# pqh22/ProxyTransformation

Hardware: AMD Instinct MI355X
Metric: scenes/sec (100k pts, 256 clusters, 64 proxies) (higher is better)
Workload: dtype f32; 1 GPU; cfg2: N=100000 pts, gs=8->M'=256 kept clusters, L=64 text + V=196 image proxies, d=256, eval forward; scenes_per_gpu=4, img_feat_dtype=bf16, input_sets_rotated=3, streams=1, lanes=1 (one forward at a time), setup_forwards=32

## Files before the change

### proxytransformation_amd/csrc/api.hip

```cpp
#include <atomic>
#include <chrono>
#include <cmath>
#include <cstdlib>
#include <cstring>
#include <mutex>
#include <utility>
#include <vector>

#include "common.h"

namespace ptx {

static thread_local char g_err[512] = "";

void set_error(const char *fmt, ...)
{
    va_list ap;
    va_start(ap, fmt);
    vsnprintf(g_err, sizeof(g_err), fmt, ap);
    va_end(ap);
}

static const char *const kKernelNames[] = {
    "k_minmax", "k_cluster", "k_select", "k_tags",
// ... 377 lines not shown
                         float *img_proxy, void *ws, hipStream_t st, int phase = 0, bool need_ln = true,
                         int i0 = 0, int ni = -1, uint32_t *gate = nullptr, uint32_t gate_seq = 0)
{
    const PrepLayout P = prep_layout(s);
    const WsLayout L = ws_layout(s);
    const int C = s.C, hd = P.hd, nall = s.B * s.V, nimg = ni < 0 ? nall : ni;
    float *fm = at<float>(ws, L.fm) + (size_t)i0 * s.in_dim, *qkv0 = at<float>(ws, L.qkv0) + (size_t)i0 * 3 * C;
    float *we = at<float>(ws, L.we) + (size_t)i0 * s.heads * P.KT1, *gbuf = at<float>(ws, L.gbuf) + (size_t)i0 * s.heads * P.KT2p;
    float *obuf = at<float>(ws, L.obuf) + (size_t)i0 * C, *cbuf = at<float>(ws, L.cbuf) + (size_t)i0 * C;
    if (img_proxy) img_proxy += (size_t)i0 * C;
    const int dt = s.img_dtype;
    img = static_cast<const char *>(img) + (size_t)i0 * s.in_dim * s.hw * (dt == 0 ? 4 : 2);
    float *Gs = nullptr, *E = nullptr, *ML = nullptr;
    const int EW = P.KT2p - s.in_dim;
    const bool pooled32 = img_pool32_supported(dt, s.in_dim, s.hw, s.heads);
    const bool pooled = pooled32 || img_pool_supported(dt, s.in_dim, s.hw, s.heads);
    if (pooled) {
        img_pool_layout(at<float>(ws, L.pool), nall, s.in_dim, EW, &Gs, &E, &ML);
        Gs += (size_t)i0 * 2 * s.heads * s.in_dim; E += (size_t)i0 * s.heads * EW; ML += (size_t)i0 * s.heads * 5;
    }
    if (phase != 2) PTX_TIMED(KID_IMG_MEAN, st, launch_img_mean(img, dt, nimg, s.in_dim, s.hw, fm, st, gate, gate_seq));
    if (phase == 1) return PTX_OK;
    const bool chained = hd == 32 && nimg < 4096;
    {
        GemmBatch g{}; g.n = 1;
        g.p[0] = GemmProb{fm, prep + P.w3, qkv0, prep + P.b3, nullptr, nullptr, nullptr,
                          nimg, 3 * C, s.in_dim, s.in_dim, s.in_dim, 3 * C, 0, 0, 0, EPI_NONE};
        if (chained) {
            g.p[0].w2 = prep + P.t1; g.p[0].c2 = we; g.p[0].n2 = P.KT1; g.p[0].ldc2 = s.heads * P.KT1;
            g.p[0].chain_tiles = s.heads; g.p[0].w2_stride = (long)P.KT1 * hd; g.p[0].c2_stride = P.KT1;
        }
        PTX_TIMED(KID_IMG_QKV0, st, launch_gemm(g, st));
    }
    if (!chained) {
        for (int h0 = 0; h0 < s.heads; h0 += kMaxGroups) {
            GemmBatch g{}; g.n = std::min(kMaxGroups, s.heads - h0);
            for (int h = h0; h < h0 + g.n; ++h)
                g.p[h - h0] = GemmProb{qkv0 + h * hd, prep + P.t1 + (size_t)h * P.KT1 * hd, we + (size_t)h * P.KT1,
                                       nullptr, nullptr, nullptr, nullptr, nimg, P.KT1, hd, 3 * C, hd,
                                       s.heads * P.KT1, 0, 0, 0, EPI_NONE};
            PTX_TIMED(KID_IMG_WE, st, launch_gemm(g, st));
        }
    }
    if (pooled32) {
        PTX_TIMED_EXT(KID_IMG_SCORES, st, launch_img_pool32(static_cast<const float *>(img), we, qkv0, nimg, s.in_dim, s.hw, C, P.KT1, EW,
                                                        attn_scale(hd), Gs, E, ML, st));
    } else if (pooled) {
        PTX_TIMED_EXT(KID_IMG_SCORES, st, launch_img_pool(img, dt, we, qkv0, nimg, s.in_dim, s.hw, C, P.KT1,
                                                      EW, attn_scale(hd), Gs, E, ML, st));
    } else {
        PTX_TIMED(KID_IMG_SCORES, st, launch_img_scores(img, dt, we, qkv0, nimg, s.in_dim, s.hw, s.heads, C, P.KT1,
                                                        P.KT2p, attn_scale(hd), gbuf, st));
        PTX_TIMED(KID_IMG_GATHER, st, launch_img_gather(img, dt, nimg, s.in_dim, s.hw, s.heads, P.KT2p, gbuf, st));
    }
    for (int h0 = 0; h0 < s.heads; h0 += kMaxGroups) {
        GemmBatch g{}; g.n = std::min(kMaxGroups, s.heads - h0);
        for (int h = h0; h < h0 + g.n; ++h) {
            GemmProb &gp = g.p[h - h0];
            gp = GemmProb{gbuf + (size_t)h * P.KT2p, prep + P.t2 + (size_t)h * hd * P.KT2p, obuf + h * hd,
                          w.v_b + h * hd, nullptr, gbuf + (size_t)h * P.KT2p + s.in_dim,
                          qkv0 + 2 * C + h * hd, nimg, hd, P.KT2p, s.heads * P.KT2p, P.KT2p, C,
                          0, s.heads * P.KT2p, 3 * C, EPI_NONE};
            if (pooled) {
                gp.A = nullptr; gp.rs = nullptr;
                gp.pg = Gs + (size_t)h * s.in_dim; gp.ldg = 2 * s.heads * s.in_dim; gp.gslab = s.heads * s.in_dim;
                gp.pe = E + (size_t)h * EW; gp.lde = s.heads * EW;
                gp.pml = ML + (size_t)h * 5; gp.ldml = s.heads * 5;
                gp.kg = s.in_dim;
            }
        }
        PTX_TIMED(KID_IMG_O, st, launch_gemm(g, st));
    }
    {
        GemmBatch g{}; g.n = 1;
        g.p[0] = GemmProb{obuf, w.c_w, cbuf, w.c_b, nullptr, nullptr, nullptr,
                          nimg, C, C, C, C, C, 0, 0, 0, EPI_NONE};
        g.p[0].lnp_out = at<float>(ws, L.lnp_img) + (size_t)i0 * (C / 32) * 2;
        PTX_TIMED(KID_IMG_C, st, launch_gemm(g, st));
    }
    if (need_ln) {
        LnBatch lb{}; lb.n = 1; lb.C = C; lb.eps = s.ln_eps;
        lb.p[0] = LnProb{cbuf, img_proxy, w.norm_img_w, w.norm_img_b, nullptr, nimg, 1};
        PTX_TIMED(KID_IMG_LN, st, launch_ln_rows(lb, st));
    }
    return PTX_OK;
}

struct Branch {
    const PtxBlock *blk; const float *x_in; const float *proxy; int Lp; const uint8_t *mask;
    const float *head_w, *head_b, *head_ab; int nout; float *head_out; float *guide; int slot;
    bool late_proxy;
// ... 797 lines not shown
```

### proxytransformation_amd/csrc/common.h

```cpp
#pragma once
#include <hip/hip_runtime.h>
#include <cstdarg>
#include <cstdint>
#include <cstdio>

#include "../../include/proxyt.h"

namespace ptx {

void set_error(const char *fmt, ...);
bool timing_ext_take(hipEvent_t *start, hipEvent_t *stop);

#define PTX_REQUIRE(cond, ...)                                   \
    do {                                                         \
        if (!(cond)) {                                           \
            ::ptx::set_error(__VA_ARGS__);                       \
            return PTX_EINVAL;                                   \
        }                                                        \
    } while (0)

#define PTX_HIP(expr)                                                              \
    do {                                                                           \
        hipError_t e_ = (expr);                                                    \
        if (e_ != hipSuccess) {                                                    \
// ... 188 lines not shown
    size_t order, picks, keep, ksrc, kcenter, kcluster, kidx, drop_idx, tile_counts;
    size_t point_proxy, x_in[2];
    size_t pp_all, xln_all[2], g_all[2];
    size_t order_e;
    size_t fm, qkv0, we, pool, gbuf, obuf, cbuf, img_proxy;
    size_t qkv[2], pt[2], pv[2], ao[2], x1[2], xn2[2], hbuf[2], x2[2], guide[2], head[2];
    size_t lnp_img, lnp_x1[2];
    size_t fa_part;
    size_t mlp_part;
    size_t total;
};
WsLayout ws_layout(const PtxShape &s);

int validate_shape(const PtxShape &s);

enum : int { EPI_NONE = 0, EPI_GELU = 1 };
struct GemmProb {
    const float *A; const float *W; float *C;
    const float *bias;
    const float *res;
    const float *rs;
    const float *ad;
    int R, N, K, lda, ldw, ldc, ldres, rs_stride, ldad, epi;
    const float *pg, *pe, *pml; int ldg, gslab, lde, ldml, kg;
    float *lnp_out;
    const float *lnp_in, *ln_c; int ln_parts, ln_C; float ln_eps;
    const float *w2; float *c2; int n2, ldc2, chain_tiles; long w2_stride, c2_stride;
};
constexpr int kMaxGroups = 8;
struct GemmBatch {
    GemmProb p[kMaxGroups]; int n; int rotate;
    GateRef tail_gate;
};
int launch_gemm(const GemmBatch &gb, hipStream_t st, int compute_dtype = 0);
int gemm_policy(int min_tiles_128);

struct LnProb { const float *x; float *y; const float *w; const float *b; const float *add; int R, add_rows; };
struct LnBatch { LnProb p[2]; int n; int C; float eps; };
int launch_ln_rows(const LnBatch &lb, hipStream_t st);

struct HeadProb {
    const float *x; const float *nw; const float *nb;
    const float *hw; const float *hb;
    const float *ab;
    float *out; float *guide; int R, nout;
};
struct HeadBatch { HeadProb p[2]; int n; int C; float eps; };
// ... 70 lines not shown
                const int32_t *keep = nullptr);
int launch_select_slots(const PtxShape &s, const int32_t *idx, const float *cluster, const int32_t *order,
                        const int32_t *picks, const int32_t *keep, float *kcluster, int32_t *kidx,
                        int32_t *drop_idx, uint32_t *tag, hipStream_t st);
int launch_t_ln_fwd(const float *x, const float *w, const float *b, int R, int C, float eps, float *y, float *stats, hipStream_t st);
int t_ln_chunks(int R);
int launch_t_ln_bwd(const float *x, const float *stats, const float *w, const float *dy, int R, int C, float *dx, float *part, hipStream_t st);
int launch_tile_count(const uint32_t *tag, int B, int N, int32_t *tile_counts, int32_t *counts, int32_t *scene_acc,
                      hipStream_t st);
int launch_affine(const PtxShape &s, const ScenePts &points, uint32_t *tag, const float *kcenter,
                  const float *translate, const float *transform, float *out, int32_t *counts,
                  const int32_t *tile_counts, bool compact, bool clear_tag, hipStream_t st,
                  const uint32_t *poison = nullptr);

int launch_img_mean(const void *img, int dt, int nimg, int in_dim, int hw, float *fm, hipStream_t st,
                    uint32_t *gate = nullptr, uint32_t gate_seq = 0);
int launch_img_scores(const void *img, int dt, const float *we, const float *qkv0, int nimg, int in_dim,
                      int hw, int heads, int C, int KT1, int KT2p, float scale, float *gbuf, hipStream_t st);
int launch_img_gather(const void *img, int dt, int nimg, int in_dim, int hw, int heads, int KT2p, float *gbuf,
                      hipStream_t st);
bool img_pool_supported(int dt, int in_dim, int hw, int heads);
size_t img_pool_bytes(int nimg, int in_dim, int EW);
void img_pool_layout(float *scratch, int nimg, int in_dim, int EW, float **Gs, float **E, float **ML);
int launch_img_pool(const void *img, int dt, const float *we, const float *qkv0, int nimg, int in_dim, int hw, int C,
                    int KT1, int EW, float scale, float *Gs, float *E, float *ML, hipStream_t st);

bool img_pool32_supported(int dt, int in_dim, int hw, int heads);
int launch_img_pool32(const float *img, const float *we, const float *qkv0, int nimg, int in_dim, int hw, int C, int KT1, int EW,
                      float scale, float *Gs, float *E, float *ML, hipStream_t st);

int run_prepare(const PtxShape &s, const PtxWeights &w, float *prep, hipStream_t st);

}
```

### proxytransformation_amd/csrc/gemm.hip

```cpp
#include <atomic>
#include <cstdlib>

#include "common.h"
#include "split3.h"
#include "mfma64.h"

namespace ptx {


__device__ __forceinline__ void pin4(float4 &v) { asm volatile("" : "+v"(v.x), "+v"(v.y), "+v"(v.z), "+v"(v.w)); }
__device__ __forceinline__ void ln_row_stats(const GemmProb &pr, int row, float &mu, float &rstd)
{
    const float2 *pp = reinterpret_cast<const float2 *>(pr.lnp_in) + (size_t)row * pr.ln_parts;
    constexpr int kMaxParts = 16;
    float2 v[kMaxParts];
#pragma unroll
    for (int t = 0; t < kMaxParts; ++t) v[t] = pp[min(t, pr.ln_parts - 1)];
    float s1 = 0.0f, s2 = 0.0f;
#pragma unroll
    for (int t = 0; t < kMaxParts; ++t) { s1 += t < pr.ln_parts ? v[t].x : 0.0f; s2 += t < pr.ln_parts ? v[t].y : 0.0f; }
    const float inv = 1.0f / (float)pr.ln_C;
    mu = s1 * inv;
    float between = 0.0f;
#pragma unroll
// ... 449 lines not shown
#undef PTX_Y_COMPUTE

template <int SK, int AMODE, bool CHAIN = false, bool LN = false>
__global__ __launch_bounds__(SK * 64) void k_gemm32(GemmBatch gb)
{
    const GemmProb pr = gb.p[blockIdx.z];
    const int row0 = blockIdx.x * 32, col0 = blockIdx.y * 32;
    if (row0 >= pr.R || col0 >= pr.N) return;
    extern __shared__ __attribute__((aligned(16))) float lds[];
    const int lane = threadIdx.x & 63;
    const int wv = __builtin_amdgcn_readfirstlane(threadIdx.x >> 6);
    float *base = lds + (size_t)wv * (4 * 32 * LDT);
    const int li = lane & 31, hh = lane >> 5;
    const int nk = (pr.K + BK - 1) / BK, per = (nk + SK - 1) / SK;
    const int it0 = wv * per, it1 = min(nk, it0 + per);
    const int r0 = lane >> 3, kq = (lane & 7) * 4;
    const size_t a0 = (size_t)min(row0 + r0, pr.R - 1) * pr.lda, a1 = (size_t)min(row0 + r0 + 8, pr.R - 1) * pr.lda;
    const size_t a2 = (size_t)min(row0 + r0 + 16, pr.R - 1) * pr.lda, a3 = (size_t)min(row0 + r0 + 24, pr.R - 1) * pr.lda;
    const size_t w0 = (size_t)min(col0 + r0, pr.N - 1) * pr.ldw, w1 = (size_t)min(col0 + r0 + 8, pr.N - 1) * pr.ldw;
    const size_t w2 = (size_t)min(col0 + r0 + 16, pr.N - 1) * pr.ldw, w3 = (size_t)min(col0 + r0 + 24, pr.N - 1) * pr.ldw;
    const float4 z4 = make_float4(0.f, 0.f, 0.f, 0.f);
    float4 aA0, aA1, aA2, aA3, wA0, wA1, wA2, wA3, aB0, aB1, aB2, aB3, wB0, wB1, wB2, wB3;
    float4 gA0 = z4, gA1 = z4, gA2 = z4, gA3 = z4, gB0 = z4, gB1 = z4, gB2 = z4, gB3 = z4;
    int kA = 0, kB = 0;
    (void)kA; (void)kB;
    size_t g0 = 0, g1 = 0, g2 = 0, g3 = 0, e0 = 0, e1 = 0, e2 = 0, e3 = 0;
    float fc0[4] = {0.f, 0.f, 0.f, 0.f}, fc1[4] = {0.f, 0.f, 0.f, 0.f}, fct[4] = {0.f, 0.f, 0.f, 0.f};
    float *cts = lds + (size_t)SK * (4 * 32 * LDT);
    float *lnst = cts + 32 + wv * 64;
    const bool ln = LN && pr.lnp_in != nullptr;
    float mu4[4] = {0.0f, 0.0f, 0.0f, 0.0f};
    if (AMODE == 1) {
#pragma unroll
        for (int i = 0; i < 4; ++i) {
            const int row = min(row0 + r0 + 8 * i, pr.R - 1);
            const float *ml = pr.pml + (size_t)row * pr.ldml;
            const float m0 = ml[0], l0 = ml[1], m1 = ml[2], l1 = ml[3], s0 = ml[4];
            const float m = fmaxf(fmaxf(m0, m1), s0);
            const float x0 = __expf(m0 - m), x1 = __expf(m1 - m), xt = __expf(s0 - m);
            const float inv = 1.0f / ((l0 * x0 + l1 * x1) + xt);
            fc0[i] = x0 * inv; fc1[i] = x1 * inv; fct[i] = xt * inv;
            if (wv == 0 && (lane & 7) == 0) cts[r0 + 8 * i] = fct[i];
        }
        g0 = (size_t)min(row0 + r0, pr.R - 1) * pr.ldg; g1 = (size_t)min(row0 + r0 + 8, pr.R - 1) * pr.ldg;
        g2 = (size_t)min(row0 + r0 + 16, pr.R - 1) * pr.ldg; g3 = (size_t)min(row0 + r0 + 24, pr.R - 1) * pr.ldg;
        e0 = (size_t)min(row0 + r0, pr.R - 1) * pr.lde; e1 = (size_t)min(row0 + r0 + 8, pr.R - 1) * pr.lde;
        e2 = (size_t)min(row0 + r0 + 16, pr.R - 1) * pr.lde; e3 = (size_t)min(row0 + r0 + 24, pr.R - 1) * pr.lde;
    }
#define PTX_FETCH(S, j_)                                                                  \
    do {                                                                                  \
        int jj_ = min((j_), cnt - 1) + rot;                                               \
        jj_ -= jj_ >= cnt ? cnt : 0;                                                      \
        const int k_ = (it0 + jj_) * BK + kq, kc_ = min(k_, pr.K - 4);                    \
        const bool ok_ = k_ < pr.K;                                                       \
        if (AMODE == 0) {                                                                 \
            a##S##0 = *reinterpret_cast<const float4 *>(pr.A + a0 + kc_);                 \
            a##S##1 = *reinterpret_cast<const float4 *>(pr.A + a1 + kc_);                 \
            a##S##2 = *reinterpret_cast<const float4 *>(pr.A + a2 + kc_);                 \
            a##S##3 = *reinterpret_cast<const float4 *>(pr.A + a3 + kc_);                 \
        } else if (kc_ < pr.kg) {               \
            a##S##0 = *reinterpret_cast<const float4 *>(pr.pg + g0 + kc_);                \
            a##S##1 = *reinterpret_cast<const float4 *>(pr.pg + g1 + kc_);                \
            a##S##2 = *reinterpret_cast<const float4 *>(pr.pg + g2 + kc_);                \
            a##S##3 = *reinterpret_cast<const float4 *>(pr.pg + g3 + kc_);                \
            g##S##0 = *reinterpret_cast<const float4 *>(pr.pg + g0 + pr.gslab + kc_);     \
            g##S##1 = *reinterpret_cast<const float4 *>(pr.pg + g1 + pr.gslab + kc_);     \
            g##S##2 = *reinterpret_cast<const float4 *>(pr.pg + g2 + pr.gslab + kc_);     \
            g##S##3 = *reinterpret_cast<const float4 *>(pr.pg + g3 + pr.gslab + kc_);     \
        } else {                                                                          \
            a##S##0 = *reinterpret_cast<const float4 *>(pr.pe + e0 + (kc_ - pr.kg));      \
            a##S##1 = *reinterpret_cast<const float4 *>(pr.pe + e1 + (kc_ - pr.kg));      \
            a##S##2 = *reinterpret_cast<const float4 *>(pr.pe + e2 + (kc_ - pr.kg));      \
            a##S##3 = *reinterpret_cast<const float4 *>(pr.pe + e3 + (kc_ - pr.kg));      \
        }                                                                                 \
        k##S = kc_;                                                                       \
        w##S##0 = *reinterpret_cast<const float4 *>(pr.W + w0 + kc_);                     \
        w##S##1 = *reinterpret_cast<const float4 *>(pr.W + w1 + kc_);                     \
        w##S##2 = *reinterpret_cast<const float4 *>(pr.W + w2 + kc_);                     \
        w##S##3 = *reinterpret_cast<const float4 *>(pr.W + w3 + kc_);                     \
        if (!ok_) { w##S##0 = z4; w##S##1 = z4; w##S##2 = z4; w##S##3 = z4; }             \
    } while (0)
#define PTX_MERGE(S, i_)                                                                  \
    do {                                                                                  \
        if (k##S < pr.kg) {                                                               \
            a##S##i_ = make_float4(a##S##i_.x * fc0[i_] + g##S##i_.x * fc1[i_], a##S##i_.y * fc0[i_] + g##S##i_.y * fc1[i_], \
                                   a##S##i_.z * fc0[i_] + g##S##i_.z * fc1[i_], a##S##i_.w * fc0[i_] + g##S##i_.w * fc1[i_]); \
        } else {                                                                          \
            const int t_ = k##S - pr.kg;       \
            a##S##i_.x *= t_ == 0 ? fct[i_] : (t_ <= 128 ? fc0[i_] : fc1[i_]);           \
            a##S##i_.y *= t_ + 1 <= 128 ? fc0[i_] : fc1[i_];                              \
            a##S##i_.z *= t_ + 2 <= 128 ? fc0[i_] : fc1[i_];                              \
            a##S##i_.w *= t_ + 3 <= 128 ? fc0[i_] : fc1[i_];                              \
        }                                                                                 \
    } while (0)
#define PTX_STASH(S, buf_)                                                                \
    do {                                                                                  \
        float *A_s = base + (buf_) * (2 * 32 * LDT) + r0 * LDT + kq, *W_s = A_s + 32 * LDT; \
        if (AMODE == 1) { PTX_MERGE(S, 0); PTX_MERGE(S, 1); PTX_MERGE(S, 2); PTX_MERGE(S, 3); } \
        if (LN) { sub4(a##S##0, mu4[0]); sub4(a##S##1, mu4[1]); sub4(a##S##2, mu4[2]); sub4(a##S##3, mu4[3]); } \
        *reinterpret_cast<float4 *>(A_s) = a##S##0;                                       \
        *reinterpret_cast<float4 *>(A_s + 8 * LDT) = a##S##1;                             \
        *reinterpret_cast<float4 *>(A_s + 16 * LDT) = a##S##2;                            \
        *reinterpret_cast<float4 *>(A_s + 24 * LDT) = a##S##3;                            \
        *reinterpret_cast<float4 *>(W_s) = w##S##0;                                       \
        *reinterpret_cast<float4 *>(W_s + 8 * LDT) = w##S##1;                             \
        *reinterpret_cast<float4 *>(W_s + 16 * LDT) = w##S##2;                            \
        *reinterpret_cast<float4 *>(W_s + 24 * LDT) = w##S##3;                            \
    } while (0)
#define PTX_COMPUTE(buf_)                                                                 \
// ... 151 lines not shown
                                    hipFuncAttributeMaxDynamicSharedMemorySize, (int)lds));
    hipLaunchKernelGGL((k_gemm32<SK, AMODE, CHAIN, LN>), dim3(cdiv(rmax, 32), cdiv(nmax, 32), gb.n), dim3(SK * 64), lds, st, gb);
    return PTX_OK;
}

static std::atomic<int> g_gemm128_min_tiles{256};
int gemm_policy(int min_tiles_128)
{
    return min_tiles_128 < 0 ? g_gemm128_min_tiles.load() : g_gemm128_min_tiles.exchange(min_tiles_128);
}

int launch_gemm(const GemmBatch &gb_in, hipStream_t st, int compute_dtype)
{
    GemmBatch gb = gb_in;
    gb.rotate = 0;
    PTX_REQUIRE(gb.n >= 1 && gb.n <= kMaxGroups, "gemm: %d groups", gb.n);
    int rmax = 0, nmax = 0, kmin = 1 << 30, kmax = 0;
    long tiles32 = 0;
    bool any_ln = false;
    for (int g = 0; g < gb.n; ++g) {
        const GemmProb &p = gb.p[g];
        PTX_REQUIRE((p.A || p.pg) && p.W && p.C, "gemm: null operand in group %d", g);
        PTX_REQUIRE((p.pg != nullptr) == (gb.p[0].pg != nullptr), "gemm: mixed A modes in one batch");
        PTX_REQUIRE(p.pg == nullptr || (p.pe && p.pml && p.ad && p.kg % BK == 0 && p.kg <= p.K && p.ldg % 4 == 0 &&
                                        p.gslab % 4 == 0 && p.lde % 4 == 0),
                    "gemm: bad pooled-A description in group %d", g);
        PTX_REQUIRE(p.R >= 1 && p.N >= 1 && p.K >= 4, "gemm: empty problem in group %d", g);
        PTX_REQUIRE(p.K % 4 == 0 && p.lda % 4 == 0 && p.ldw % 4 == 0,
                    "gemm: K=%d lda=%d ldw=%d must be multiples of 4", p.K, p.lda, p.ldw);
        PTX_REQUIRE(((reinterpret_cast<uintptr_t>(p.A) | reinterpret_cast<uintptr_t>(p.W) | reinterpret_cast<uintptr_t>(p.pg) |
                      reinterpret_cast<uintptr_t>(p.pe)) & 15) == 0,
                    "gemm: operands of group %d are not 16-byte aligned", g);
        PTX_REQUIRE(p.rs == nullptr || p.ad != nullptr, "gemm: row scale without addend");
        PTX_REQUIRE(p.lnp_in == nullptr || (p.ln_c && p.ln_parts >= 1 && p.ln_parts <= 16 && p.ln_C == 32 * p.ln_parts &&
                                            p.K == p.ln_C && p.pg == nullptr && p.bias == nullptr),
                    "gemm: bad LayerNorm-consumer description in group %d", g);
        any_ln = any_ln || p.lnp_in != nullptr;
        rmax = p.R > rmax ? p.R : rmax;
        nmax = p.N > nmax ? p.N : nmax;
        kmin = p.K < kmin ? p.K : kmin;
        kmax = p.K > kmax ? p.K : kmax;
        tiles32 += (long)cdiv(p.R, 32) * cdiv(p.N, 32);
    }
    if (gb.p[0].w2 != nullptr) {
        PTX_REQUIRE(gb.n == 1 && gb.p[0].pg == nullptr && gb.p[0].c2 && gb.p[0].n2 >= 1 && gb.p[0].chain_tiles >= 1 &&
                    gb.p[0].chain_tiles * 32 <= gb.p[0].N && gb.p[0].K >= 4 * BK && gb.p[0].lnp_out == nullptr && !any_ln,
                    "gemm: bad chained-product description");
        PTX_TRY((launch_gemm32<4, 0, true>(gb, rmax, nmax, st)));
// ... 202 lines not shown
```

### proxytransformation_amd/csrc/imgpool.hip

```cpp
#include <cstdlib>
#include <hip/hip_ext.h>

#include "common.h"
#include "imgstore.h"

namespace ptx {

typedef __bf16 bf16x8 __attribute__((ext_vector_type(8)));

constexpr int kPoolHeads = 8;
constexpr int kPoolNtImages = 4096;
constexpr int kPoolWPad = 544;
constexpr int kPoolPPad = 136;

typedef _Float16 f16x8 __attribute__((ext_vector_type(8)));

template <int DT>
__device__ __forceinline__ void split3(float x, unsigned short &q1, unsigned short &q2, unsigned short &q3)
{
    if (DT == 1) {
        const unsigned int u1 = __float_as_uint(x) & 0xffff0000u;
        const float r1 = x - __uint_as_float(u1);
        const unsigned int u2 = __float_as_uint(r1) & 0xffff0000u;
        const float r2 = r1 - __uint_as_float(u2);
// ... 22 lines not shown
    return (amax > 0.0f && e > -100 && e < 100) ? 13 - e : 0;
}
__device__ __forceinline__ float pow2f(int k) { return __uint_as_float((unsigned int)(127 + k) << 23); }
constexpr float kPoolEScale = 16384.0f;

__device__ __forceinline__ u32x4 shr_elems(const u32x4 &v, int k)
{
    const int ws = k >> 1;
    unsigned int w[8] = {v[0], v[1], v[2], v[3], 0u, 0u, 0u, 0u};
    u32x4 o;
#pragma unroll
    for (int q = 0; q < 4; ++q) {
        unsigned int lo = 0u, hi = 0u;
#pragma unroll
        for (int s = 0; s < 4; ++s) {
            if (ws == s) { lo = w[q + s]; hi = w[q + s + 1]; }
        }
        o[q] = (k & 1) ? ((lo >> 16) | (hi << 16)) : lo;
    }
    return o;
}

struct PoolArgs {
    const unsigned short *img; const float *we, *qkv0;
    int nimg, in_dim, hw, C, KT1, EW; float scale;
    float *Gs;
    float *E;
    float *ML;
};

template <int DT, bool NT>
__global__ __launch_bounds__(512) void k_img_pool(PoolArgs a)
{
    constexpr int heads = kPoolHeads;
    extern __shared__ __attribute__((aligned(16))) unsigned char smem[];
    float *partial = reinterpret_cast<float *>(smem);
    unsigned short *wpart = reinterpret_cast<unsigned short *>(partial + 8 * heads * 128);
    unsigned short *parts = wpart + 24 * kPoolWPad;
    const int in_dim = a.in_dim, hw = a.hw;
    const int xcd = blockIdx.x & 7, slot = blockIdx.x >> 3;
    const int T = slot & 1, imr = (slot >> 1) * 8 + xcd;
    if (imr >= a.nimg) return;
    const int im = a.nimg - 1 - imr;
    const int slab = im * 2 + T;
    const int tid = threadIdx.x, lane = lane_id();
    const int wid = __builtin_amdgcn_readfirstlane(tid >> 6);
    const int n = lane & 15, kq = lane >> 4;
    const float *wim = a.we + (size_t)im * heads * a.KT1;
    const unsigned short *f = a.img + (size_t)im * in_dim * hw;
    const int px = 128 * T + 8 * n;
    const bool full = px + 8 <= hw;
    const int cw = 64 * wid;
    float wv[heads];
#pragma unroll
    for (int h = 0; h < heads; ++h) wv[h] = wim[(size_t)h * a.KT1 + tid];
    u32x4 L[2][8];
    const bool tensor_end = im == a.nimg - 1 && cw + 64 == in_dim;
#pragma unroll
    for (int kb = 0; kb < 2; ++kb) {
        const unsigned short *r = f + (size_t)(cw + 32 * kb + 8 * kq) * hw + px;
#pragma unroll
        for (int i = 0; i < 8; ++i) {
            if (kb == 1 && i == 7 && tensor_end) {
                const bool lastrow = kq == 3 && !full;
                const int back = lastrow ? px + 8 - hw : 0;
                const int bk = back > 8 ? px - (hw - 8) : back;
                u32x4 v = __builtin_nontemporal_load(reinterpret_cast<const u4u2 *>(r + (size_t)i * hw - bk));
                L[kb][i] = lastrow ? (back >= 8 ? u32x4{0u, 0u, 0u, 0u} : shr_elems(v, back)) : v;
            } else {
                L[kb][i] = __builtin_nontemporal_load(reinterpret_cast<const u4u2 *>(r + (size_t)i * hw));
            }
        }
    }
    float ev[2];
#pragma unroll
    for (int u = 0; u < 2; ++u) {
        const int p = 128 * T + lane + 64 * u;
        ev[u] = p < hw ? wim[(size_t)wid * a.KT1 + in_dim + 1 + p] : 0.0f;
    }
    float sq = 0.0f, sk = 0.0f;
    if (T == 0) {
        const int hd = a.C / heads;
        const float *qv = a.qkv0 + (size_t)im * 3 * a.C + wid * hd;
        if (lane < hd) { sq = qv[lane]; sk = qv[a.C + lane]; }
    }
    {
        const int c = tid;
#pragma unroll
        for (int h = 0; h < heads; ++h) {
            if (DT == 2) {
                const int k = pow2_scale_exp(wave_max(fabsf(wv[h])));
                wv[h] *= pow2f(k);
                if (lane == 0) *reinterpret_cast<float *>(wpart + (size_t)h * kPoolWPad + in_dim + 2 * wid) = pow2f(-k);
            }
            unsigned short q1, q2, q3;
            split3<DT>(wv[h], q1, q2, q3);
            wpart[(size_t)h * kPoolWPad + c] = q1;
            wpart[(size_t)(8 + h) * kPoolWPad + c] = q2;
            wpart[(size_t)(16 + h) * kPoolWPad + c] = q3;
        }
    }
    __syncthreads();

    {
        f32x4 acc[8];
#pragma unroll
        for (int j = 0; j < 8; ++j) acc[j] = f32x4{0.f, 0.f, 0.f, 0.f};
        const bool lo = n < heads;
#pragma unroll
        for (int kb = 0; kb < 2; ++kb) {
// ... 24 lines not shown
                *reinterpret_cast<float4 *>(d + 4) = make_float4(acc[4][r] * us, acc[5][r] * us, acc[6][r] * us, acc[7][r] * us);
            }
        }
    }
    __syncthreads();

    {
        const int h = wid;
        float e[2], mloc = -INFINITY, sv[2];
#pragma unroll
        for (int u = 0; u < 2; ++u) {
            const int p = lane + 64 * u;
            float s = 0.0f;
#pragma unroll
            for (int w = 0; w < 8; ++w) s += partial[((size_t)w * heads + h) * 128 + p];
            sv[u] = 128 * T + p < hw ? s + ev[u] : -INFINITY;
            mloc = fmaxf(mloc, sv[u]);
        }
        const float m = wave_max(mloc);
#pragma unroll
        for (int u = 0; u < 2; ++u) e[u] = 128 * T + lane + 64 * u < hw ? expf(sv[u] - m) : 0.0f;
        const float l = wave_sum(e[0] + e[1]);
        float *erow = a.E + ((size_t)im * heads + h) * a.EW;
        const float s0 = T == 0 ? wave_sum(sq * sk) * a.scale : 0.0f;
        if (lane == 0) {
            float *ml = a.ML + ((size_t)im * heads + h) * 5;
            ml[2 * T] = m;
            ml[2 * T + 1] = l;
            if (T == 0) { ml[4] = s0; erow[0] = 1.0f; }
        }
#pragma unroll
        for (int u = 0; u < 2; ++u) {
            const int p = lane + 64 * u;
            const int t = 1 + 128 * T + p;
            if (t <= hw || (T == (hw > 128 ? 1 : 0) && t < a.EW)) erow[t] = t <= hw ? e[u] : 0.0f;
            unsigned short q1, q2, q3;
            split3<DT>(DT == 2 ? e[u] * kPoolEScale : e[u], q1, q2, q3);
            parts[(size_t)h * kPoolPPad + p] = q1;
            parts[(size_t)(8 + h) * kPoolPPad + p] = q2;
            parts[(size_t)(16 + h) * kPoolPPad + p] = q3;
        }
    }
    __syncthreads();

    {
        const int ps = n & 3, hh = n >> 2;
        const int src = ((ps + 4 * kq) + 16 * (n >> 2)) * 4;
// ... 57 lines not shown
            if (NT) asm volatile("global_store_dwordx4 %0, %1, off sc1 nt" :: "v"(dst + i), "v"(v) : "memory");
            else    asm volatile("global_store_dwordx4 %0, %1, off sc1" :: "v"(dst + i), "v"(v) : "memory");
        }
    }
}

bool img_pool_supported(int dt, int in_dim, int hw, int heads)
{
    return (dt == 1 || dt == 2) && heads == kPoolHeads && in_dim == 512 && hw > 128 && hw <= 255;
}

size_t img_pool_bytes(int nimg, int in_dim, int EW)
{
    return (size_t)nimg * kPoolHeads * (2 * (size_t)in_dim + EW + 8) * sizeof(float);
}

void img_pool_layout(float *scratch, int nimg, int in_dim, int EW, float **Gs, float **E, float **ML)
{
    *Gs = scratch;
    *E = *Gs + (size_t)nimg * 2 * kPoolHeads * in_dim;
    *ML = *E + (size_t)nimg * kPoolHeads * EW;
}

int launch_img_pool(const void *img, int dt, const float *we, const float *qkv0, int nimg, int in_dim, int hw, int C,
                    int KT1, int EW, float scale, float *Gs, float *E, float *ML, hipStream_t st)
{
    PTX_REQUIRE(EW % 4 == 0 && EW >= hw + 1 && hw > 128 && hw <= 255, "img pool: hw=%d EW=%d", hw, EW);
    PoolArgs pa{static_cast<const unsigned short *>(img), we, qkv0, nimg, in_dim, hw, C, KT1, EW, scale, Gs, E, ML};
    const size_t lds = sizeof(float) * 8 * kPoolHeads * 128 + sizeof(unsigned short) * 24 * (kPoolWPad + kPoolPPad);
    PTX_REQUIRE(lds <= 64 * 1024, "img pool: %zu B of LDS", lds);
    static const int nt_env = getenv("PTX_POOL_NT") ? atoi(getenv("PTX_POOL_NT")) : -1;
    const bool nt = nt_env >= 0 ? nt_env != 0 : nimg >= kPoolNtImages;
    const dim3 grid(cdiv(nimg, 8) * 16);
    hipEvent_t ta = nullptr, tb = nullptr;
    (void)timing_ext_take(&ta, &tb);
    if (dt == 1) { if (nt) hipExtLaunchKernelGGL((k_img_pool<1, true>), grid, dim3(512), lds, st, ta, tb, 0, pa); else hipExtLaunchKernelGGL((k_img_pool<1, false>), grid, dim3(512), lds, st, ta, tb, 0, pa); }
    else         { if (nt) hipExtLaunchKernelGGL((k_img_pool<2, true>), grid, dim3(512), lds, st, ta, tb, 0, pa); else hipExtLaunchKernelGGL((k_img_pool<2, false>), grid, dim3(512), lds, st, ta, tb, 0, pa); }
    PTX_LAUNCHED("k_img_pool");
    return PTX_OK;
}

}
```

### proxytransformation_amd/csrc/imgpool32.hip

```cpp
#include <hip/hip_ext.h>

#include "common.h"

namespace ptx {

typedef float p32_f4u __attribute__((ext_vector_type(4), aligned(4)));
typedef float p32_f4 __attribute__((ext_vector_type(4)));

constexpr int kP32Heads = 8;
constexpr int kP32Tile = 32;
constexpr int kP32Tiles = 128 / kP32Tile;
constexpr int kP32TRow = 36;

struct Pool32Args {
    const float *img; const float *we, *qkv0;
    int nimg, in_dim, hw, C, KT1, EW; float scale;
    float *Gs, *E, *ML;
};

__global__ __launch_bounds__(512) __attribute__((amdgpu_waves_per_eu(4, 4))) void k_img_pool32(Pool32Args a)
{
    constexpr int heads = kP32Heads, TP = kP32Tile;
    extern __shared__ __attribute__((aligned(16))) float p32_sm[];
    float *W_s = p32_sm;
    float *S_s = W_s + 512 * heads;
    float *E_s = S_s + 8 * heads * TP;
    float *sc_s = E_s + heads * TP;
    float *T_s = sc_s + 16;
    const int in_dim = a.in_dim, hw = a.hw;
    const int xcd = blockIdx.x & 7, slot = blockIdx.x >> 3;
    const int H = slot & 1, imr = (slot >> 1) * 8 + xcd;
    if (imr >= a.nimg) return;
    const int im = a.nimg - 1 - imr;
    const int tid = threadIdx.x, lane = lane_id();
    const int wid = __builtin_amdgcn_readfirstlane(tid >> 6);
    const int n = lane & 7, kq = lane >> 3;
    const int mr = lane & 15, mk = lane >> 4;
    const float *wim = a.we + (size_t)im * heads * a.KT1;
    const float *f = a.img + (size_t)im * in_dim * hw;
    float *T_w = T_s + (size_t)wid * (16 * kP32TRow);
    float wv[heads];
#pragma unroll
    for (int h = 0; h < heads; ++h) wv[h] = wim[(size_t)h * a.KT1 + tid];
    float ev[kP32Tiles];
#pragma unroll
    for (int t = 0; t < kP32Tiles; ++t) {
        const int p = 128 * H + TP * t + (lane & (TP - 1));
        ev[t] = p < hw ? wim[(size_t)wid * a.KT1 + in_dim + 1 + p] : 0.0f;
    }
    float sq = 0.0f, sk = 0.0f;
    if (H == 0) {
        const int hd = a.C / heads;
        const float *qv = a.qkv0 + (size_t)im * 3 * a.C + wid * hd;
        if (lane < hd) { sq = qv[lane]; sk = qv[a.C + lane]; }
    }
    const char *fb = reinterpret_cast<const char *>(f);
    const unsigned row_off = (unsigned)(64 * wid + kq) * (unsigned)hw * 4u, row_step = 8u * (unsigned)hw * 4u;
    const bool tensor_end = im == a.nimg - 1 && wid == 7 && kq == 7;
    {
        *reinterpret_cast<p32_f4 *>(W_s + tid * heads) = p32_f4{wv[0], wv[1], wv[2], wv[3]};
        *reinterpret_cast<p32_f4 *>(W_s + tid * heads + 4) = p32_f4{wv[4], wv[5], wv[6], wv[7]};
        if (tid < 16) sc_s[tid] = 0.0f;
    }
    p32_f4 D[4];
#pragma unroll
    for (int q = 0; q < 4; ++q) D[q] = p32_f4{0.f, 0.f, 0.f, 0.f};
    float m_run = -INFINITY, l_run = 0.0f, e_t[kP32Tiles];
#pragma unroll
    for (int t = 0; t < kP32Tiles; ++t) e_t[t] = 0.0f;

#pragma unroll
    for (int t = 0; t < kP32Tiles; ++t) {
        const int px0 = 128 * H + TP * t;
        p32_f4u L[8];
        {
            const int p = px0 + 4 * n;
            const int pc = p < hw ? p : 0;
            const unsigned off0 = row_off + (unsigned)pc * 4u;
#pragma unroll
            for (int i = 0; i < 8; ++i) {
                const float *rowp = reinterpret_cast<const float *>(fb + (off0 + (unsigned)i * row_step)) - pc;
                if (i == 7 && tensor_end && pc + 4 > hw) {
                    const p32_f4u v = *reinterpret_cast<const p32_f4u *>(rowp + hw - 4);
                    const int back = pc + 4 - hw;
                    L[i] = back == 1 ? p32_f4u{v[1], v[2], v[3], 0.f} : back == 2 ? p32_f4u{v[2], v[3], 0.f, 0.f} : p32_f4u{v[3], 0.f, 0.f, 0.f};
// ... 39 lines not shown
        {
            const int h = wid, pl = lane & (TP - 1);
            float s = 0.0f;
#pragma unroll
            for (int w = 0; w < 8; ++w) s += S_s[((size_t)w * heads + h) * TP + pl];
            const bool valid = lane < TP && px0 + pl < hw;
            const float sv = valid ? s + ev[t] : -INFINITY;
            const float m_new = fmaxf(m_run, wave_max(sv));
            const float resc = expf(m_run - m_new);
            const float e = valid ? expf(sv - m_new) : 0.0f;
            l_run = l_run * resc + wave_sum(e);
            m_run = m_new;
#pragma unroll
            for (int u = 0; u < kP32Tiles; ++u) e_t[u] = u < t ? e_t[u] * resc : (u == t ? e : 0.0f);
            if (lane < TP) E_s[h * TP + lane] = e;
            if (lane == 0) sc_s[h] = resc;
            if (t == kP32Tiles - 1) {
                float *erow = a.E + ((size_t)im * heads + h) * a.EW;
#pragma unroll
                for (int u = 0; u < kP32Tiles; ++u) {
                    const int tok = 1 + 128 * H + TP * u + lane;
                    if (lane < TP && tok < a.EW) erow[tok] = e_t[u];
                }
                const float s0 = H == 0 ? wave_sum(sq * sk) * a.scale : 0.0f;
                if (lane == 0) {
                    float *ml = a.ML + ((size_t)im * heads + h) * 5;
                    ml[2 * H] = m_run; ml[2 * H + 1] = l_run;
                    if (H == 0) { ml[4] = s0; erow[0] = 1.0f; }
                }
            }
        }
        __syncthreads();
        {
            const float resc = sc_s[mr];
#pragma unroll
            for (int q = 0; q < 4; ++q) { D[q][0] *= resc; D[q][1] *= resc; D[q][2] *= resc; D[q][3] *= resc; }
#pragma unroll
            for (int q = 0; q < 4; ++q) {
#pragma unroll
                for (int ii = 0; ii < 2; ++ii)
                    *reinterpret_cast<p32_f4 *>(T_w + (8 * ii + kq) * kP32TRow + 4 * n) = p32_f4{L[2 * q + ii][0], L[2 * q + ii][1], L[2 * q + ii][2], L[2 * q + ii][3]};
                __builtin_amdgcn_wave_barrier();
                __builtin_amdgcn_fence(__ATOMIC_RELEASE, "wavefront");
#pragma unroll
                for (int pb = 0; pb < TP / 16; ++pb) {
                    const p32_f4 a4 = *reinterpret_cast<const p32_f4 *>(T_w + mr * kP32TRow + 16 * pb + 4 * mk);
                    p32_f4 e4 = *reinterpret_cast<const p32_f4 *>(E_s + (mr & 7) * TP + 16 * pb + 4 * mk);
// ... 8 lines not shown
    }
    __syncthreads();
    float *G = W_s;
    if (mr < heads) {
#pragma unroll
        for (int q = 0; q < 4; ++q)
            *reinterpret_cast<p32_f4 *>(G + (size_t)mr * in_dim + 64 * wid + 16 * q + 4 * mk) = D[q];
    }
    __syncthreads();
    {
        float *dst = a.Gs + (size_t)(im * 2 + H) * heads * in_dim;
        for (int i = tid * 4; i < heads * in_dim; i += 512 * 4) {
            const p32_f4 v = *reinterpret_cast<const p32_f4 *>(G + i);
            asm volatile("global_store_dwordx4 %0, %1, off sc1" :: "v"(dst + i), "v"(v) : "memory");
        }
    }
}

bool img_pool32_supported(int dt, int in_dim, int hw, int heads)
{
    return dt == 0 && heads == kP32Heads && in_dim == 512 && hw > 128 && hw <= 255;
}

int launch_img_pool32(const float *img, const float *we, const float *qkv0, int nimg, int in_dim, int hw, int C, int KT1, int EW,
                      float scale, float *Gs, float *E, float *ML, hipStream_t st)
{
    PTX_REQUIRE(EW % 4 == 0 && EW >= hw + 1 && hw > 128 && hw <= 255 && in_dim == 512, "img pool (fp32): hw=%d EW=%d in_dim=%d", hw, EW, in_dim);
    PTX_REQUIRE((reinterpret_cast<uintptr_t>(img) & 15) == 0, "img_feat must be 16-byte aligned");
    Pool32Args pa{img, we, qkv0, nimg, in_dim, hw, C, KT1, EW, scale, Gs, E, ML};
    const size_t lds = sizeof(float) * (512 * kP32Heads + 8 * kP32Heads * kP32Tile + kP32Heads * kP32Tile + 16 + 8 * 16 * kP32TRow);
    const dim3 grid(cdiv(nimg, 8) * 16);
    hipEvent_t ta = nullptr, tb = nullptr;
    (void)timing_ext_take(&ta, &tb);
    hipExtLaunchKernelGGL(k_img_pool32, grid, dim3(512), lds, st, ta, tb, 0, pa);
    PTX_LAUNCHED("k_img_pool32");
    return PTX_OK;
}

}
```

### proxytransformation_amd/csrc/prep.hip

```cpp
#include "common.h"

namespace ptx {

__global__ void k_prep_bn(const float *w, const float *b, const float *mean, const float *var,
                          int n, float eps, float *ab)
{
    const int i = blockIdx.x * blockDim.x + threadIdx.x;
    if (i >= n) return;
    const float alpha = w[i] / sqrtf(var[i] + eps);
    ab[i] = alpha;
    ab[n + i] = b[i] - mean[i] * alpha;
}

__global__ void k_prep_posbias(const float *pb, const float *pc, const float *pr, int Mk, int s, int C,
                               float *out)
{
    const int i = blockIdx.x * blockDim.x + threadIdx.x;
    if (i >= Mk * C) return;
    const int j = i / C, yx = i - j * C, y = yx / s, x = yx - y * s;
    const float sc = 4.0f / (float)s;
    float sy = sc * ((float)y + 0.5f) - 0.5f; if (sy < 0.f) sy = 0.f;
    float sx = sc * ((float)x + 0.5f) - 0.5f; if (sx < 0.f) sx = 0.f;
    const int y0 = (int)sy, x0 = (int)sx;
    const int y1 = y0 + (y0 < 3 ? 1 : 0), x1 = x0 + (x0 < 3 ? 1 : 0);
// ... 14 lines not shown
    const int part = n / C, r = n - part * C;
    const float *wrow = (part == 0 ? qw : (part == 1 ? kw : vw)) + (size_t)r * C;
    float s = 0.0f;
    if (c < in_dim) {
        for (int j = 0; j < C; ++j) s = fmaf(wrow[j], cw[(size_t)j * in_dim + c], s);
        w3[(size_t)n * in_dim + c] = s;
    } else {
        for (int j = 0; j < C; ++j) s = fmaf(wrow[j], cb[j] + pos[j], s);
        b3[n] = s + (part == 0 ? qb[r] : 0.0f);
    }
}

__global__ void k_prep_t1(const float *kw, const float *cw, const float *cb, const float *pos, int C,
                          int in_dim, int hw, int heads, float scale, float *t1)
{
    const int hd = C / heads, KT1 = in_dim + hw + 1;
    const int i = blockIdx.x * blockDim.x + threadIdx.x;
    if (i >= heads * KT1 * hd) return;
    const int h = i / (KT1 * hd), rem = i - h * KT1 * hd, t = rem / hd, d = rem - t * hd;
    const float *wk = kw + (size_t)(h * hd + d) * C;
    float s = 0.0f;
    if (t < in_dim) {
        for (int j = 0; j < C; ++j) s = fmaf(wk[j], cw[(size_t)j * in_dim + t], s);
    } else if (t > in_dim) {
        const float *pi = pos + (size_t)(t - in_dim) * C;
        for (int j = 0; j < C; ++j) s = fmaf(wk[j], cb[j] + pi[j], s);
    }
    t1[i] = s * scale;
}

__global__ void k_prep_t2(const float *vw, const float *cw, const float *cb, const float *pos, int C,
                          int in_dim, int hw, int heads, int KT2p, float *t2)
{
    const int hd = C / heads;
    const int i = blockIdx.x * blockDim.x + threadIdx.x;
    if (i >= heads * hd * KT2p) return;
    const int h = i / (hd * KT2p), rem = i - h * hd * KT2p, d = rem / KT2p, t = rem - d * KT2p;
    const float *wv = vw + (size_t)(h * hd + d) * C;
    float s = 0.0f;
    if (t < in_dim) {
        for (int j = 0; j < C; ++j) s = fmaf(wv[j], cw[(size_t)j * in_dim + t], s);
    } else if (t > in_dim && t <= in_dim + hw) {
        const float *pi = pos + (size_t)(t - in_dim) * C;
        for (int j = 0; j < C; ++j) s = fmaf(wv[j], cb[j] + pi[j], s);
    }
    t2[i] = s;
}
// ... 78 lines not shown
```

Baseline: 18820 scenes/s.

## Drop K/V columns from img QKV0 GEMM by folding into pooled kernels

When the pooled image-attention path is taken, the first QKV GEMM now computes only the Q columns instead of all 3C outputs. The self-score term s0 (q·k for the mean token) is rebuilt inside the pool kernels from folded weights (t1 row in_dim now holds the bias/pos term) dotted with the mean feature fm. The V contribution of the mean token is recomputed in the O GEMM's merge step from fm and a bias vector. This removes two-thirds of that GEMM's work and its qkv0 reads, at the cost of extra wave reductions, extra LDS, and extra fm loads in the O GEMM.

```diff
diff --git a/proxytransformation_amd/csrc/api.hip b/proxytransformation_amd/csrc/api.hip
--- a/proxytransformation_amd/csrc/api.hip
+++ b/proxytransformation_amd/csrc/api.hip
@@ -423,10 +423,11 @@
     if (phase != 2) PTX_TIMED(KID_IMG_MEAN, st, launch_img_mean(img, dt, nimg, s.in_dim, s.hw, fm, st, gate, gate_seq));
     if (phase == 1) return PTX_OK;
     const bool chained = hd == 32 && nimg < 4096;
+    const int n0 = pooled ? C : 3 * C;
     {
         GemmBatch g{}; g.n = 1;
         g.p[0] = GemmProb{fm, prep + P.w3, qkv0, prep + P.b3, nullptr, nullptr, nullptr,
-                          nimg, 3 * C, s.in_dim, s.in_dim, s.in_dim, 3 * C, 0, 0, 0, EPI_NONE};
+                          nimg, n0, s.in_dim, s.in_dim, s.in_dim, 3 * C, 0, 0, 0, EPI_NONE};
         if (chained) {
             g.p[0].w2 = prep + P.t1; g.p[0].c2 = we; g.p[0].n2 = P.KT1; g.p[0].ldc2 = s.heads * P.KT1;
             g.p[0].chain_tiles = s.heads; g.p[0].w2_stride = (long)P.KT1 * hd; g.p[0].c2_stride = P.KT1;
@@ -444,11 +445,11 @@
         }
     }
     if (pooled32) {
-        PTX_TIMED_EXT(KID_IMG_SCORES, st, launch_img_pool32(static_cast<const float *>(img), we, qkv0, nimg, s.in_dim, s.hw, C, P.KT1, EW,
-                                                        attn_scale(hd), Gs, E, ML, st));
+        PTX_TIMED_EXT(KID_IMG_SCORES, st, launch_img_pool32(static_cast<const float *>(img), we, fm, nimg, s.in_dim, s.hw, P.KT1, EW,
+                                                        Gs, E, ML, st));
     } else if (pooled) {
-        PTX_TIMED_EXT(KID_IMG_SCORES, st, launch_img_pool(img, dt, we, qkv0, nimg, s.in_dim, s.hw, C, P.KT1,
-                                                      EW, attn_scale(hd), Gs, E, ML, st));
+        PTX_TIMED_EXT(KID_IMG_SCORES, st, launch_img_pool(img, dt, we, fm, nimg, s.in_dim, s.hw, P.KT1,
+                                                      EW, Gs, E, ML, st));
     } else {
         PTX_TIMED(KID_IMG_SCORES, st, launch_img_scores(img, dt, we, qkv0, nimg, s.in_dim, s.hw, s.heads, C, P.KT1,
                                                         P.KT2p, attn_scale(hd), gbuf, st));
@@ -468,6 +469,8 @@
                 gp.pe = E + (size_t)h * EW; gp.lde = s.heads * EW;
                 gp.pml = ML + (size_t)h * 5; gp.ldml = s.heads * 5;
                 gp.kg = s.in_dim;
+                gp.pfm = fm; gp.ldfm = s.in_dim;
+                gp.ad = prep + P.b3 + 2 * C + h * hd; gp.ldad = 0;
             }
         }
         PTX_TIMED(KID_IMG_O, st, launch_gemm(g, st));
diff --git a/proxytransformation_amd/csrc/common.h b/proxytransformation_amd/csrc/common.h
--- a/proxytransformation_amd/csrc/common.h
+++ b/proxytransformation_amd/csrc/common.h
@@ -234,7 +234,7 @@
     const float *rs;
     const float *ad;
     int R, N, K, lda, ldw, ldc, ldres, rs_stride, ldad, epi;
-    const float *pg, *pe, *pml; int ldg, gslab, lde, ldml, kg;
+    const float *pg, *pe, *pml, *pfm; int ldg, gslab, lde, ldml, kg, ldfm;
     float *lnp_out;
     const float *lnp_in, *ln_c; int ln_parts, ln_C; float ln_eps;
     const float *w2; float *c2; int n2, ldc2, chain_tiles; long w2_stride, c2_stride;
@@ -351,12 +351,12 @@
 bool img_pool_supported(int dt, int in_dim, int hw, int heads);
 size_t img_pool_bytes(int nimg, int in_dim, int EW);
 void img_pool_layout(float *scratch, int nimg, int in_dim, int EW, float **Gs, float **E, float **ML);
-int launch_img_pool(const void *img, int dt, const float *we, const float *qkv0, int nimg, int in_dim, int hw, int C,
-                    int KT1, int EW, float scale, float *Gs, float *E, float *ML, hipStream_t st);
+int launch_img_pool(const void *img, int dt, const float *we, const float *fm, int nimg, int in_dim, int hw,
+                    int KT1, int EW, float *Gs, float *E, float *ML, hipStream_t st);
 
 bool img_pool32_supported(int dt, int in_dim, int hw, int heads);
-int launch_img_pool32(const float *img, const float *we, const float *qkv0, int nimg, int in_dim, int hw, int C, int KT1, int EW,
-                      float scale, float *Gs, float *E, float *ML, hipStream_t st);
+int launch_img_pool32(const float *img, const float *we, const float *fm, int nimg, int in_dim, int hw, int KT1, int EW,
+                      float *Gs, float *E, float *ML, hipStream_t st);
 
 int run_prepare(const PtxShape &s, const PtxWeights &w, float *prep, hipStream_t st);
 
diff --git a/proxytransformation_amd/csrc/gemm.hip b/proxytransformation_amd/csrc/gemm.hip
--- a/proxytransformation_amd/csrc/gemm.hip
+++ b/proxytransformation_amd/csrc/gemm.hip
@@ -495,9 +495,10 @@
     const float4 z4 = make_float4(0.f, 0.f, 0.f, 0.f);
     float4 aA0, aA1, aA2, aA3, wA0, wA1, wA2, wA3, aB0, aB1, aB2, aB3, wB0, wB1, wB2, wB3;
     float4 gA0 = z4, gA1 = z4, gA2 = z4, gA3 = z4, gB0 = z4, gB1 = z4, gB2 = z4, gB3 = z4;
+    float4 fA0 = z4, fA1 = z4, fA2 = z4, fA3 = z4, fB0 = z4, fB1 = z4, fB2 = z4, fB3 = z4;
     int kA = 0, kB = 0;
     (void)kA; (void)kB;
-    size_t g0 = 0, g1 = 0, g2 = 0, g3 = 0, e0 = 0, e1 = 0, e2 = 0, e3 = 0;
+    size_t g0 = 0, g1 = 0, g2 = 0, g3 = 0, e0 = 0, e1 = 0, e2 = 0, e3 = 0, f0 = 0, f1 = 0, f2 = 0, f3 = 0;
     float fc0[4] = {0.f, 0.f, 0.f, 0.f}, fc1[4] = {0.f, 0.f, 0.f, 0.f}, fct[4] = {0.f, 0.f, 0.f, 0.f};
     float *cts = lds + (size_t)SK * (4 * 32 * LDT);
     float *lnst = cts + 32 + wv * 64;
@@ -519,6 +520,8 @@
         g2 = (size_t)min(row0 + r0 + 16, pr.R - 1) * pr.ldg; g3 = (size_t)min(row0 + r0 + 24, pr.R - 1) * pr.ldg;
         e0 = (size_t)min(row0 + r0, pr.R - 1) * pr.lde; e1 = (size_t)min(row0 + r0 + 8, pr.R - 1) * pr.lde;
         e2 = (size_t)min(row0 + r0 + 16, pr.R - 1) * pr.lde; e3 = (size_t)min(row0 + r0 + 24, pr.R - 1) * pr.lde;
+        f0 = (size_t)min(row0 + r0, pr.R - 1) * pr.ldfm; f1 = (size_t)min(row0 + r0 + 8, pr.R - 1) * pr.ldfm;
+        f2 = (size_t)min(row0 + r0 + 16, pr.R - 1) * pr.ldfm; f3 = (size_t)min(row0 + r0 + 24, pr.R - 1) * pr.ldfm;
     }
 #define PTX_FETCH(S, j_)                                                                  \
     do {                                                                                  \
@@ -540,6 +543,10 @@
             g##S##1 = *reinterpret_cast<const float4 *>(pr.pg + g1 + pr.gslab + kc_);     \
             g##S##2 = *reinterpret_cast<const float4 *>(pr.pg + g2 + pr.gslab + kc_);     \
             g##S##3 = *reinterpret_cast<const float4 *>(pr.pg + g3 + pr.gslab + kc_);     \
+            f##S##0 = *reinterpret_cast<const float4 *>(pr.pfm + f0 + kc_);               \
+            f##S##1 = *reinterpret_cast<const float4 *>(pr.pfm + f1 + kc_);               \
+            f##S##2 = *reinterpret_cast<const float4 *>(pr.pfm + f2 + kc_);               \
+            f##S##3 = *reinterpret_cast<const float4 *>(pr.pfm + f3 + kc_);               \
         } else {                                                                          \
             a##S##0 = *reinterpret_cast<const float4 *>(pr.pe + e0 + (kc_ - pr.kg));      \
             a##S##1 = *reinterpret_cast<const float4 *>(pr.pe + e1 + (kc_ - pr.kg));      \
@@ -556,8 +563,11 @@
 #define PTX_MERGE(S, i_)                                                                  \
     do {                                                                                  \
         if (k##S < pr.kg) {                                                               \
-            a##S##i_ = make_float4(a##S##i_.x * fc0[i_] + g##S##i_.x * fc1[i_], a##S##i_.y * fc0[i_] + g##S##i_.y * fc1[i_], \
-                                   a##S##i_.z * fc0[i_] + g##S##i_.z * fc1[i_], a##S##i_.w * fc0[i_] + g##S##i_.w * fc1[i_]); \
+             \
+            a##S##i_ = make_float4((a##S##i_.x * fc0[i_] + g##S##i_.x * fc1[i_]) + f##S##i_.x * fct[i_], \
+                                   (a##S##i_.y * fc0[i_] + g##S##i_.y * fc1[i_]) + f##S##i_.y * fct[i_], \
+                                   (a##S##i_.z * fc0[i_] + g##S##i_.z * fc1[i_]) + f##S##i_.z * fct[i_], \
+                                   (a##S##i_.w * fc0[i_] + g##S##i_.w * fc1[i_]) + f##S##i_.w * fct[i_]); \
         } else {                                                                          \
             const int t_ = k##S - pr.kg;       \
             a##S##i_.x *= t_ == 0 ? fct[i_] : (t_ <= 128 ? fc0[i_] : fc1[i_]);           \
@@ -755,8 +765,9 @@
         const GemmProb &p = gb.p[g];
         PTX_REQUIRE((p.A || p.pg) && p.W && p.C, "gemm: null operand in group %d", g);
         PTX_REQUIRE((p.pg != nullptr) == (gb.p[0].pg != nullptr), "gemm: mixed A modes in one batch");
-        PTX_REQUIRE(p.pg == nullptr || (p.pe && p.pml && p.ad && p.kg % BK == 0 && p.kg <= p.K && p.ldg % 4 == 0 &&
-                                        p.gslab % 4 == 0 && p.lde % 4 == 0),
+        PTX_REQUIRE(p.pg == nullptr || (p.pe && p.pml && p.pfm && p.ad && p.kg % BK == 0 && p.kg <= p.K && p.ldg % 4 == 0 &&
+                                        p.gslab % 4 == 0 && p.lde % 4 == 0 && p.ldfm % 4 == 0 &&
+                                        (reinterpret_cast<uintptr_t>(p.pfm) & 15) == 0),
                     "gemm: bad pooled-A description in group %d", g);
         PTX_REQUIRE(p.R >= 1 && p.N >= 1 && p.K >= 4, "gemm: empty problem in group %d", g);
         PTX_REQUIRE(p.K % 4 == 0 && p.lda % 4 == 0 && p.ldw % 4 == 0,
diff --git a/proxytransformation_amd/csrc/imgpool.hip b/proxytransformation_amd/csrc/imgpool.hip
--- a/proxytransformation_amd/csrc/imgpool.hip
+++ b/proxytransformation_amd/csrc/imgpool.hip
@@ -68,8 +68,8 @@
 }
 
 struct PoolArgs {
-    const unsigned short *img; const float *we, *qkv0;
-    int nimg, in_dim, hw, C, KT1, EW; float scale;
+    const unsigned short *img; const float *we, *fm;
+    int nimg, in_dim, hw, KT1, EW;
     float *Gs;
     float *E;
     float *ML;
@@ -100,6 +100,8 @@
     float wv[heads];
 #pragma unroll
     for (int h = 0; h < heads; ++h) wv[h] = wim[(size_t)h * a.KT1 + tid];
+    float fmv = 0.0f;
+    if (T == 0) fmv = a.fm[(size_t)im * in_dim + tid];
     u32x4 L[2][8];
     const bool tensor_end = im == a.nimg - 1 && cw + 64 == in_dim;
 #pragma unroll
@@ -124,14 +126,17 @@
         const int p = 128 * T + lane + 64 * u;
         ev[u] = p < hw ? wim[(size_t)wid * a.KT1 + in_dim + 1 + p] : 0.0f;
     }
-    float sq = 0.0f, sk = 0.0f;
-    if (T == 0) {
-        const int hd = a.C / heads;
-        const float *qv = a.qkv0 + (size_t)im * 3 * a.C + wid * hd;
-        if (lane < hd) { sq = qv[lane]; sk = qv[a.C + lane]; }
-    }
+    float e0 = 0.0f;
+    if (T == 0) e0 = wim[(size_t)wid * a.KT1 + in_dim];
     {
         const int c = tid;
+        if (T == 0) {
+#pragma unroll
+            for (int h = 0; h < heads; ++h) {
+                const float part = wave_sum(wv[h] * fmv);
+                if (lane == 0) *reinterpret_cast<float *>(wpart + (size_t)(8 + h) * kPoolWPad + in_dim + 2 * wid) = part;
+            }
+        }
 #pragma unroll
         for (int h = 0; h < heads; ++h) {
             if (DT == 2) {
@@ -202,7 +207,12 @@
         for (int u = 0; u < 2; ++u) e[u] = 128 * T + lane + 64 * u < hw ? expf(sv[u] - m) : 0.0f;
         const float l = wave_sum(e[0] + e[1]);
         float *erow = a.E + ((size_t)im * heads + h) * a.EW;
-        const float s0 = T == 0 ? wave_sum(sq * sk) * a.scale : 0.0f;
+        float s0 = 0.0f;
+        if (T == 0) {
+#pragma unroll
+            for (int w = 0; w < 8; ++w) s0 += *reinterpret_cast<const float *>(wpart + (size_t)(8 + h) * kPoolWPad + in_dim + 2 * w);
+            s0 += e0;
+        }
         if (lane == 0) {
             float *ml = a.ML + ((size_t)im * heads + h) * 5;
             ml[2 * T] = m;
@@ -306,11 +316,11 @@
     *ML = *E + (size_t)nimg * kPoolHeads * EW;
 }
 
-int launch_img_pool(const void *img, int dt, const float *we, const float *qkv0, int nimg, int in_dim, int hw, int C,
-                    int KT1, int EW, float scale, float *Gs, float *E, float *ML, hipStream_t st)
+int launch_img_pool(const void *img, int dt, const float *we, const float *fm, int nimg, int in_dim, int hw,
+                    int KT1, int EW, float *Gs, float *E, float *ML, hipStream_t st)
 {
     PTX_REQUIRE(EW % 4 == 0 && EW >= hw + 1 && hw > 128 && hw <= 255, "img pool: hw=%d EW=%d", hw, EW);
-    PoolArgs pa{static_cast<const unsigned short *>(img), we, qkv0, nimg, in_dim, hw, C, KT1, EW, scale, Gs, E, ML};
+    PoolArgs pa{static_cast<const unsigned short *>(img), we, fm, nimg, in_dim, hw, KT1, EW, Gs, E, ML};
     const size_t lds = sizeof(float) * 8 * kPoolHeads * 128 + sizeof(unsigned short) * 24 * (kPoolWPad + kPoolPPad);
     PTX_REQUIRE(lds <= 64 * 1024, "img pool: %zu B of LDS", lds);
     static const int nt_env = getenv("PTX_POOL_NT") ? atoi(getenv("PTX_POOL_NT")) : -1;
diff --git a/proxytransformation_amd/csrc/imgpool32.hip b/proxytransformation_amd/csrc/imgpool32.hip
--- a/proxytransformation_amd/csrc/imgpool32.hip
+++ b/proxytransformation_amd/csrc/imgpool32.hip
@@ -13,8 +13,8 @@
 constexpr int kP32TRow = 36;
 
 struct Pool32Args {
-    const float *img; const float *we, *qkv0;
-    int nimg, in_dim, hw, C, KT1, EW; float scale;
+    const float *img; const float *we, *fm;
+    int nimg, in_dim, hw, KT1, EW;
     float *Gs, *E, *ML;
 };
 
@@ -27,6 +27,7 @@
     float *E_s = S_s + 8 * heads * TP;
     float *sc_s = E_s + heads * TP;
     float *T_s = sc_s + 16;
+    float *M_s = T_s + 8 * 16 * kP32TRow;
     const int in_dim = a.in_dim, hw = a.hw;
     const int xcd = blockIdx.x & 7, slot = blockIdx.x >> 3;
     const int H = slot & 1, imr = (slot >> 1) * 8 + xcd;
@@ -42,17 +43,13 @@
     float wv[heads];
 #pragma unroll
     for (int h = 0; h < heads; ++h) wv[h] = wim[(size_t)h * a.KT1 + tid];
+    float fmv = 0.0f, e0 = 0.0f;
+    if (H == 0) { fmv = a.fm[(size_t)im * in_dim + tid]; e0 = wim[(size_t)wid * a.KT1 + in_dim]; }
     float ev[kP32Tiles];
 #pragma unroll
     for (int t = 0; t < kP32Tiles; ++t) {
         const int p = 128 * H + TP * t + (lane & (TP - 1));
         ev[t] = p < hw ? wim[(size_t)wid * a.KT1 + in_dim + 1 + p] : 0.0f;
-    }
-    float sq = 0.0f, sk = 0.0f;
-    if (H == 0) {
-        const int hd = a.C / heads;
-        const float *qv = a.qkv0 + (size_t)im * 3 * a.C + wid * hd;
-        if (lane < hd) { sq = qv[lane]; sk = qv[a.C + lane]; }
     }
     const char *fb = reinterpret_cast<const char *>(f);
     const unsigned row_off = (unsigned)(64 * wid + kq) * (unsigned)hw * 4u, row_step = 8u * (unsigned)hw * 4u;
@@ -61,6 +58,13 @@
         *reinterpret_cast<p32_f4 *>(W_s + tid * heads) = p32_f4{wv[0], wv[1], wv[2], wv[3]};
         *reinterpret_cast<p32_f4 *>(W_s + tid * heads + 4) = p32_f4{wv[4], wv[5], wv[6], wv[7]};
         if (tid < 16) sc_s[tid] = 0.0f;
+        if (H == 0) {
+#pragma unroll
+            for (int h = 0; h < heads; ++h) {
+                const float part = wave_sum(wv[h] * fmv);
+                if (lane == 0) M_s[h * 8 + wid] = part;
+            }
+        }
     }
     p32_f4 D[4];
 #pragma unroll
@@ -146,7 +150,12 @@
                     const int tok = 1 + 128 * H + TP * u + lane;
                     if (lane < TP && tok < a.EW) erow[tok] = e_t[u];
                 }
-                const float s0 = H == 0 ? wave_sum(sq * sk) * a.scale : 0.0f;
+                float s0 = 0.0f;
+                if (H == 0) {
+#pragma unroll
+                    for (int w = 0; w < 8; ++w) s0 += M_s[h * 8 + w];
+                    s0 += e0;
+                }
                 if (lane == 0) {
                     float *ml = a.ML + ((size_t)im * heads + h) * 5;
                     ml[2 * H] = m_run; ml[2 * H + 1] = l_run;
@@ -201,13 +210,13 @@
     return dt == 0 && heads == kP32Heads && in_dim == 512 && hw > 128 && hw <= 255;
 }
 
-int launch_img_pool32(const float *img, const float *we, const float *qkv0, int nimg, int in_dim, int hw, int C, int KT1, int EW,
-                      float scale, float *Gs, float *E, float *ML, hipStream_t st)
+int launch_img_pool32(const float *img, const float *we, const float *fm, int nimg, int in_dim, int hw, int KT1, int EW,
+                      float *Gs, float *E, float *ML, hipStream_t st)
 {
     PTX_REQUIRE(EW % 4 == 0 && EW >= hw + 1 && hw > 128 && hw <= 255 && in_dim == 512, "img pool (fp32): hw=%d EW=%d in_dim=%d", hw, EW, in_dim);
     PTX_REQUIRE((reinterpret_cast<uintptr_t>(img) & 15) == 0, "img_feat must be 16-byte aligned");
-    Pool32Args pa{img, we, qkv0, nimg, in_dim, hw, C, KT1, EW, scale, Gs, E, ML};
-    const size_t lds = sizeof(float) * (512 * kP32Heads + 8 * kP32Heads * kP32Tile + kP32Heads * kP32Tile + 16 + 8 * 16 * kP32TRow);
+    Pool32Args pa{img, we, fm, nimg, in_dim, hw, KT1, EW, Gs, E, ML};
+    const size_t lds = sizeof(float) * (512 * kP32Heads + 8 * kP32Heads * kP32Tile + kP32Heads * kP32Tile + 16 + 8 * 16 * kP32TRow + 8 * kP32Heads);
     const dim3 grid(cdiv(nimg, 8) * 16);
     hipEvent_t ta = nullptr, tb = nullptr;
     (void)timing_ext_take(&ta, &tb);
diff --git a/proxytransformation_amd/csrc/prep.hip b/proxytransformation_amd/csrc/prep.hip
--- a/proxytransformation_amd/csrc/prep.hip
+++ b/proxytransformation_amd/csrc/prep.hip
@@ -60,7 +60,7 @@
     float s = 0.0f;
     if (t < in_dim) {
         for (int j = 0; j < C; ++j) s = fmaf(wk[j], cw[(size_t)j * in_dim + t], s);
-    } else if (t > in_dim) {
+    } else {
         const float *pi = pos + (size_t)(t - in_dim) * C;
         for (int j = 0; j < C; ++j) s = fmaf(wk[j], cb[j] + pi[j], s);
     }
```

After: 18500 scenes/s. 0.983x the previous value.
